# debbiemarkslab/EVcouplings

Measured on NVIDIA H100. Metric: PLM gradient evals/s as N*L^2*q cell-ops/s, higher is better.
Workload: dtype f32 parameters/accumulation; tensor-core products as bf16 hi+lo pairs (16 mantissa bits)

## Files before the change

evcouplings_b200/_lib.py:

```python
import ctypes
import os

_HERE = os.path.dirname(os.path.abspath(__file__))
LIB_PATH = os.path.join(_HERE, "csrc", "libevcplm.so")
ABI_VERSION = 2


class EngineUnavailableError(RuntimeError):
    """libevcplm.so (the sm_90a CUDA engine) is missing / unloadable / has no device."""


class EngineError(RuntimeError):
    """A libevcplm call returned non-zero."""


c_void_p = ctypes.c_void_p
c_i32 = ctypes.c_int32
c_i64 = ctypes.c_int64
c_f32 = ctypes.c_float
c_f64 = ctypes.c_double


class FitParams(ctypes.Structure):
    _fields_ = [("max_iterations", c_i32), ("m", c_i32), ("epsilon", c_f32), ("lambda_h", c_f32),
# ... 49 lines not shown
    "evc_msa_encode": (ctypes.c_int, [c_void_p, c_i64, c_i64, c_void_p, c_void_p, c_i64, c_void_p, c_void_p, c_void_p]),
    "evc_identities_to_seq": (ctypes.c_int, [c_void_p, c_void_p, c_i64, c_i32, c_void_p, c_void_p]),
    "evc_plm_create": (ctypes.c_int, [c_void_p, c_void_p, c_i64, c_i32, c_i32, c_i32, c_void_p, c_i32]),
    "evc_plm_create_alphabet": (ctypes.c_int, [c_void_p, c_void_p, c_i64, c_i32, c_i32, c_i32, c_void_p, c_i32]),
    "evc_plm_destroy": (None, [c_void_p]),
    "evc_plm_num_params": (c_i64, [c_void_p]),
    "evc_plm_eval_data": (ctypes.c_int, [c_void_p, c_void_p, c_void_p, c_void_p, c_void_p]),
    "evc_plm_set_backward": (ctypes.c_int, [c_void_p, c_i32]),
    "evc_plm_set_forward": (ctypes.c_int, [c_void_p, c_i32]),
    "evc_plm_set_precision": (ctypes.c_int, [c_void_p, c_i32]),
    "evc_plm_set_seq_chunk": (ctypes.c_int, [c_void_p, c_i64]),
    "evc_plm_tc_bytes": (ctypes.c_int, [c_i64, c_i32, c_i32, c_i32, c_i64, c_i32, c_void_p]),
    "evc_plm_tc_bytes_alphabet": (ctypes.c_int, [c_i64, c_i32, c_i32, c_i32, c_i64, c_i32, c_void_p]),
    "evc_plm_device_bytes": (c_i64, [c_void_p]),
    "evc_plm_copy_onehot": (ctypes.c_int, [c_void_p, c_void_p, c_i64]),
    "evc_fit_workspace_bytes": (c_i64, [c_i64, c_i32]),
    "evc_plm_set_host_history": (ctypes.c_int, [c_void_p, c_i32]),
    "evc_fit_workspace_split_bytes": (ctypes.c_int, [c_i64, c_i32, c_i32, c_void_p, c_void_p]),
    "evc_plm_host_bytes": (ctypes.c_int, [c_void_p, c_void_p, c_void_p]),
    "evc_fit_default_params": (None, [c_void_p]),
    "evc_plm_fit": (ctypes.c_int, [c_void_p, c_void_p, c_void_p, c_void_p, c_void_p, c_void_p, c_void_p, c_void_p,
                                   c_void_p]),
    "evc_plm_fit_checkpointed": (ctypes.c_int, [c_void_p, c_void_p, c_void_p, c_void_p, c_void_p, c_void_p, c_void_p,
                                                c_void_p, c_void_p, c_f64, c_void_p, c_void_p, c_void_p]),
    "evc_plm_fit_prepare": (ctypes.c_int, [c_void_p, c_i32]),
    "evc_plm_fit_vector": (ctypes.c_int, [c_void_p, c_i32, c_i32, c_void_p]),
    "evc_plm_pack_fx": (ctypes.c_int, [c_void_p, c_void_p, c_void_p]),
    "evc_plm_unpack_fx": (ctypes.c_int, [c_void_p, c_void_p, c_void_p]),
    "evc_plm_set_profiling": (ctypes.c_int, [c_void_p, c_i32]),
    "evc_plm_last_stage_ms": (ctypes.c_int, [c_void_p, c_void_p]),
# ... 59 lines not shown
```

evcouplings_b200/csrc/api.cu:

```cuda
#include "../../include/evcplm.h"

#include <stdlib.h>

#include <algorithm>
#include <new>
#include <string>
#include <vector>

#include "common.cuh"
#include "internal.h"

namespace evc {
static thread_local std::string g_err;
void set_error(const std::string &msg) { g_err = msg; }
}

using namespace evc;

static cudaStream_t as_stream(void *s) { return reinterpret_cast<cudaStream_t>(s); }

static const char SUPPORTED_Q[] =
    "supported: 2 <= q <= 32 states with the gap as a state, 2 <= q <= 31 with the ignored gap coded q; "
    "every code must be below 32, the 5 bit-planes of the Hamming pass";

// ... 400 lines not shown
    const bool tcf = h->fwd_mode == 1;
    const bool tcff = h->fwd_mode == 2;
    const int single = h->precision == 1 ? 1 : 0;
    void *rt_lo = single ? nullptr : h->d_rt_lo;
    float *gJ = d_g + (int64_t)g.L * g.q;
    if (tc && h->tc.n_chunks > 1) {
        if (!tcf) {
            set_error("evc_plm_eval_data: sequence chunks need the tensor-core forward (evc_plm_set_forward 1)");
            return 1;
        }
        h->ev_valid = false;
        if (plm_tcf_expand(g, h->tcf, d_x, h->d_wt_hi, h->d_wt_lo, single, st)) return 1;
        for (int c = 0; c < h->tc.n_chunks; c++) {
            const int64_t n0 = (int64_t)c * h->tc.C, nreal = std::min(h->tc.C, g.N - n0);
            if (plm_tcf_build_xsp(g, h->tcf, h->d_msa4, h->d_x1h, n0, st)) return 1;
            if (plm_tc_build_xt(g, h->tc, h->d_msa4, h->d_xt, n0, st)) return 1;
            if (plm_tcf_logits(g, h->tcf, h->tcf_maps, h->d_x1h, h->d_zt, single, nreal, st)) return 1;
            if (plm_tcf_softmax(g, h->tcf, h->d_zt, d_x, h->d_msa4, h->d_wts, h->d_rt_hi, rt_lo, h->tc.Kp,
                                h->d_gh_part2, h->d_fx_part2, n0, nreal, st))
                return 1;
            if (plm_tc_backward(g, h->tc, h->tc_maps, h->d_Gd, single, c, st)) return 1;
        }
        if (plm_tc_finalize_pairs(g, h->tc, h->d_Gd, h->tc.planes, gJ, 1.0f, st)) return 1;
        return plm_finalize_fields_n(g, h->d_gh_part2, h->d_fx_part2, d_g, d_fx, h->tcf.ntiles_s, st);
    }
    if (!tc || (!tcf && !tcff)) {
        if (require_gather_q(h, "evc_plm_eval_data") || ensure_gather(h)) return 1;
    }
    if (prof) EVC_CUDA(cudaEventRecord(h->ev[0], st));
    if (tcff) {
        if (plm_tcff_expand(g, h->tcff, d_x, h->d_wp_hi, h->d_wp_lo, single, st)) return 1;
        if (prof) EVC_CUDA(cudaEventRecord(h->ev[1], st));
        if (plm_tcff_forward(g, h->tcff, h->tcff_maps, d_x, h->d_msa4, h->d_wts, h->d_rt_hi, h->d_rt_lo, h->tc.Kp,
                             h->d_gh_part3, h->d_fx_part3, single, st))
            return 1;
        if (prof) {
            EVC_CUDA(cudaEventRecord(h->ev[2], st));
            EVC_CUDA(cudaEventRecord(h->ev[3], st));
        }
        if (plm_tc_backward(g, h->tc, h->tc_maps, h->d_Gd, single, 0, st)) return 1;
        if (prof) EVC_CUDA(cudaEventRecord(h->ev[4], st));
        if (plm_tc_finalize_pairs(g, h->tc, h->d_Gd, h->tc.planes, gJ, 1.0f, st)) return 1;
        if (plm_finalize_fields_n(g, h->d_gh_part3, h->d_fx_part3, d_g, d_fx, h->tcff.ntile_part, st)) return 1;
    } else if (tcf) {
        if (plm_tcf_expand(g, h->tcf, d_x, h->d_wt_hi, h->d_wt_lo, single, st)) return 1;
        if (prof) EVC_CUDA(cudaEventRecord(h->ev[1], st));
        if (plm_tcf_logits(g, h->tcf, h->tcf_maps, h->d_x1h, h->d_zt, single, g.N, st)) return 1;
        if (prof) EVC_CUDA(cudaEventRecord(h->ev[2], st));
        if (plm_tcf_softmax(g, h->tcf, h->d_zt, d_x, h->d_msa4, h->d_wts, h->d_rt_hi, rt_lo, h->tc.Kp,
                            h->d_gh_part2, h->d_fx_part2, 0, g.N, st))
            return 1;
        if (prof) EVC_CUDA(cudaEventRecord(h->ev[3], st));
        if (plm_tc_backward(g, h->tc, h->tc_maps, h->d_Gd, single, 0, st)) return 1;
        if (prof) EVC_CUDA(cudaEventRecord(h->ev[4], st));
        if (plm_tc_finalize_pairs(g, h->tc, h->d_Gd, h->tc.planes, gJ, 1.0f, st)) return 1;
        if (plm_finalize_fields_n(g, h->d_gh_part2, h->d_fx_part2, d_g, d_fx, h->tcf.ntiles_s, st)) return 1;
    } else {
        if (plm_expand(g, d_x, h->d_W, st)) return 1;
        if (!tc) EVC_CUDA(cudaMemsetAsync(h->d_G, 0, (size_t)g.w_floats() * sizeof(float), st));
        if (prof) EVC_CUDA(cudaEventRecord(h->ev[1], st));
        if (plm_forward(g, h->d_W, d_x, h->d_msa4, h->d_wts, h->d_R, tc ? h->d_rt_hi : nullptr,
                        tc ? h->d_rt_lo : nullptr, h->tc.Kp, h->d_gh_part, h->d_fx_part, st))
            return 1;
        if (prof) {
            EVC_CUDA(cudaEventRecord(h->ev[2], st));
            EVC_CUDA(cudaEventRecord(h->ev[3], st));
        }
        if (tc) {
            if (plm_tc_backward(g, h->tc, h->tc_maps, h->d_Gd, single, 0, st)) return 1;
            if (prof) EVC_CUDA(cudaEventRecord(h->ev[4], st));
            if (plm_tc_finalize_pairs(g, h->tc, h->d_Gd, h->tc.planes, gJ, 1.0f, st)) return 1;
            if (plm_finalize_fields(g, h->d_gh_part, h->d_fx_part, d_g, d_fx, st)) return 1;
        } else {
            if (plm_backward(g, h->d_R, h->d_perm, h->d_bstart, h->d_G, st)) return 1;
            if (prof) EVC_CUDA(cudaEventRecord(h->ev[4], st));
            if (plm_finalize(g, h->d_G, h->d_gh_part, h->d_fx_part, d_g, gJ, d_fx, 1.0f, st)) return 1;
        }
    }
    if (prof) {
        EVC_CUDA(cudaEventRecord(h->ev[5], st));
        h->ev_valid = true;
    }
    return 0;
}
// ... 8 lines not shown
        int sm_count = 0;
        EVC_CUDA(cudaDeviceGetAttribute(&sm_count, cudaDevAttrMultiProcessorCount, h->device));
        plm_tc_geometry(h->g, sm_count, h->seq_chunk, h->tc);
        const PlmTcGeom &t = h->tc;
        const TcBwdBytes b(t);
        if (!dalloc(h, &h->d_xt, b.xt) || !dalloc(h, &h->d_rt_hi, b.rt) || !dalloc(h, &h->d_rt_lo, b.rt) ||
            !dalloc(h, &h->d_Gd, b.gd)) {
            set_error(std::string("evc_plm_set_backward: device allocation failed: ") +
                      cudaGetErrorString(cudaGetLastError()));
            return 1;
        }
        EVC_CUDA(cudaMemset(h->d_xt, 0, b.xt));
        EVC_CUDA(cudaMemset(h->d_rt_hi, 0, b.rt));
        EVC_CUDA(cudaMemset(h->d_rt_lo, 0, b.rt));
        EVC_CUDA(cudaMemset(h->d_Gd, 0, b.gd));
        if (t.n_chunks == 1 && plm_tc_build_xt(h->g, t, h->d_msa4, h->d_xt, 0, 0)) return 1;
        EVC_CUDA(cudaDeviceSynchronize());
        h->tc_maps = aligned_alloc(64, round_up((int64_t)plm_tc_map_bytes(), 64));
        if (!h->tc_maps) { set_error("evc_plm_set_backward: out of host memory"); return 1; }
        if (plm_tc_make_maps(t, h->d_xt, h->d_rt_hi, h->d_rt_lo, h->tc_maps)) return 1;
    }
    h->bwd_mode = mode;
    return 0;
}

int evc_plm_set_forward(evc_plm_t *h, int32_t mode)
{
    if (!h) { set_error("evc_plm_set_forward: null handle"); return 1; }
    if (mode < 0 || mode > 2) {
        set_error("evc_plm_set_forward: mode must be 0 (gather), 1 (tensor core) or 2 (tensor core, fused softmax)");
        return 1;
    }
    if (mode == 0 && require_gather_q(h, "evc_plm_set_forward")) return 1;
    EVC_CUDA(cudaSetDevice(h->device));
    const int64_t chunk = plm_seq_chunk_round(h->seq_chunk);
// ... 119 lines not shown
int evc_plm_copy_onehot(const evc_plm_t *h, void *host_dst, int64_t bytes)
{
    if (!h || !host_dst) { set_error("evc_plm_copy_onehot: null pointer"); return 1; }
    if (!h->d_x1h) { set_error("evc_plm_copy_onehot: the handle has no tensor-core forward (evc_plm_set_forward)"); return 1; }
    const int64_t have = h->tcf.Xrows * h->tcf.Kw * 2;
    if (bytes != have) {
        set_error("evc_plm_copy_onehot: bytes must be the operand's allocation, " + std::to_string(have));
        return 1;
    }
    EVC_CUDA(cudaSetDevice(h->device));
    EVC_CUDA(cudaDeviceSynchronize());
    EVC_CUDA(cudaMemcpy(host_dst, h->d_x1h, (size_t)bytes, cudaMemcpyDeviceToHost));
    return 0;
}

int64_t evc_fit_workspace_bytes(int64_t n, int32_t m) { return n > 0 && m > 0 ? fit_work_bytes(n, m) : -1; }

int evc_fit_workspace_split_bytes(int64_t n, int32_t m, int32_t host_pairs, int64_t *device_bytes,
                                  int64_t *host_bytes)
{
    if (!device_bytes || !host_bytes) { set_error("evc_fit_workspace_split_bytes: null pointer"); return 1; }
    if (n <= 0 || m < 1 || m > 32 || host_pairs < 0 || host_pairs > m) {
        set_error("evc_fit_workspace_split_bytes: invalid arguments (need n >= 1, 1 <= m <= 32, "
                  "0 <= host_pairs <= m)");
        return 1;
    }
    fit_work_bytes(n, m, host_pairs, device_bytes, host_bytes);
    return 0;
}

// ... 67 lines not shown
    EVC_CUDA(cudaMemcpyAsync(fx_out, h->d_fx_tmp, 2 * sizeof(double), cudaMemcpyDeviceToHost, 0));
    EVC_CUDA(cudaStreamSynchronize(0));
    return 0;
}

int evc_plm_weighted_counts(evc_plm_t *h, float *d_fi_counts, float *d_fij_counts, void *stream)
{
    if (!h || !d_fi_counts || !d_fij_counts) { set_error("evc_plm_weighted_counts: null pointer"); return 1; }
    cudaStream_t st = as_stream(stream);
    const PlmGeom &g = h->g;
    if (h->bwd_mode == 1 && h->d_gh_part2) {
        const int ntiles = h->tcf.ntiles_s;
        const PlmTcGeom &t = h->tc;
        for (int c = 0; c < t.n_chunks; c++) {
            const int64_t n0 = (int64_t)c * t.C, nreal = std::min(t.C, g.N - n0);
            if (t.n_chunks > 1 && plm_tc_build_xt(g, t, h->d_msa4, h->d_xt, n0, st)) return 1;
            if (plm_tc_onehot_residual(g, ntiles, h->d_msa4, h->d_wts, h->d_rt_hi, h->d_rt_lo, t.Kp, h->d_gh_part2,
                                       h->d_fx_part2, n0, nreal, st))
                return 1;
            if (plm_tc_backward(g, t, h->tc_maps, h->d_Gd, 0, c, st)) return 1;
        }
        if (plm_tc_finalize_pairs(g, t, h->d_Gd, t.planes, d_fij_counts, 0.5f, st)) return 1;
        return plm_finalize_fields_n(g, h->d_gh_part2, nullptr, d_fi_counts, nullptr, ntiles, st);
    }
    if (require_gather_q(h, "evc_plm_weighted_counts") || ensure_gather(h)) return 1;
    EVC_CUDA(cudaMemsetAsync(h->d_G, 0, (size_t)g.w_floats() * sizeof(float), st));
    if (plm_onehot_residual(g, h->d_msa4, h->d_wts, h->d_R, h->d_gh_part, st)) return 1;
    if (plm_backward(g, h->d_R, h->d_perm, h->d_bstart, h->d_G, st)) return 1;
    return plm_finalize(g, h->d_G, h->d_gh_part, nullptr, d_fi_counts, d_fij_counts, nullptr, 0.5f, st);
}

int evc_ec_scores(const float *d_J_tri, const float *d_fij_tri, const float *d_fi, int32_t L, int32_t q,
                  float *d_fn_raw, float *d_fn_zero_sum, float *d_mi, void *stream)
{
    if (!d_J_tri) { set_error("evc_ec_scores: null pointer"); return 1; }
// ... 53 lines not shown
```

evcouplings_b200/csrc/internal.h:

```cpp
#pragma once
#include <cuda_runtime.h>
#include <stdint.h>

namespace evc {

int64_t hamming_plane_words(int64_t N, int L);
int64_t hamming_num_tiles(int64_t N);
int hamming_pack(const uint8_t *d_codes, int64_t N, int L, uint32_t *d_planes, cudaStream_t st);
int hamming_count_tiles(const uint32_t *d_planes, const int *d_mult, int64_t N, int L, int min_identical,
                        int64_t tile_begin, int64_t tile_end, int *d_counts, cudaStream_t st);

int identities_to_seq(const uint8_t *d_codes, const uint8_t *d_seq, int64_t N, int L, int *d_out, cudaStream_t st);

int msa_unique(const uint8_t *d_codes, int64_t N, int L, int *d_first, int *d_inverse, int *d_mult, int64_t *U_out,
               cudaStream_t st);

struct PlmGeom {
    int64_t N;
    int L;
    int Lp;
    int q;
    int QB;
    int S;
    int gap_code;
// ... 39 lines not shown
    int n_chunks;
    int64_t Mp;
    int64_t Np;
    int64_t Kp;
    int ksplit;
    int ksplit_last;
    int planes;
    int64_t kp_chunk(int c, int64_t N) const
    {
        const int64_t n = N - (int64_t)c * C < C ? N - (int64_t)c * C : C;
        return (n + 63) / 64 * 64;
    }
};
void plm_tc_geometry(const PlmGeom &g, int sm_count, int64_t seq_chunk, PlmTcGeom &t);
size_t plm_tc_map_bytes();
int plm_tc_build_xt(const PlmGeom &g, const PlmTcGeom &t, const uint32_t *d_msa4, void *d_xt, int64_t n0,
                    cudaStream_t st);
int plm_tc_make_maps(const PlmTcGeom &t, void *d_xt, void *d_rt_hi, void *d_rt_lo, void *maps_out_host);
int plm_tc_backward(const PlmGeom &g, const PlmTcGeom &t, const void *maps_host, float *d_Gd, int single, int chunk,
                    cudaStream_t st);
int plm_tc_onehot_residual(const PlmGeom &g, int ntiles, const uint32_t *d_msa4, const float *d_wts, void *d_rt_hi,
                           void *d_rt_lo, int64_t Kp, float *d_gh_part, double *d_fx_part, int64_t n0, int64_t nreal,
                           cudaStream_t st);
int plm_tc_finalize_pairs(const PlmGeom &g, const PlmTcGeom &t, const float *d_Gd, int planes, float *d_gJ,
                          float scale, cudaStream_t st);
struct PlmTcfGeom {
    int64_t Mp;
    int64_t Kw;
    int64_t Ns;
    int64_t Xrows;
    int ntiles_s;
};
void plm_tcf_geometry(const PlmGeom &g, const PlmTcGeom &tc, PlmTcfGeom &t);
int plm_tcf_build_x(const PlmGeom &g, const PlmTcfGeom &t, const uint32_t *d_msa4, void *d_x1h, int64_t n0,
                    cudaStream_t st);
// ... 107 lines not shown
```

evcouplings_b200/csrc/plm_tc.cu:

```cuda
#include <cuda.h>
#include <cuda_bf16.h>

#include <stdlib.h>

#include <algorithm>

#include "common.cuh"
#include "internal.h"

namespace evc {

constexpr int TC_BM = 128;
constexpr int TC_BN = 192;
constexpr int TC_BK = 64;
constexpr int TC_MAX_STAGES = 8;
constexpr int TC_A_BYTES = TC_BM * TC_BK * 2;
constexpr int TC_B_BYTES = TC_BN * TC_BK * 2;
constexpr int TC_SMEM_LIMIT = 232448;
constexpr int TC_SMEM_HEAD = 2048;
constexpr int TC_THREADS = 384;
constexpr int TC_CONSUMERS = 256;
constexpr int TC_K_CHUNK = 32;
constexpr int TC_MAX_KSPLIT = 8;
constexpr int TC_REG_PRODUCER = 40;
constexpr int TC_REG_CONSUMER = 232;

__device__ __forceinline__ void mbar_wait_bounded(uint64_t *bar, uint32_t parity)
{
    uint32_t done = 0;
    for (uint64_t it = 0; it < (1ull << 31); it++) {
        asm volatile(
            "{\n.reg .pred p;\n"
// ... 144 lines not shown
        : "+f"(d[0]), "+f"(d[1]), "+f"(d[2]), "+f"(d[3]), "+f"(d[4]), "+f"(d[5]), "+f"(d[6]), "+f"(d[7]),
          "+f"(d[8]), "+f"(d[9]), "+f"(d[10]), "+f"(d[11]), "+f"(d[12]), "+f"(d[13]), "+f"(d[14]), "+f"(d[15]),
          "+f"(d[16]), "+f"(d[17]), "+f"(d[18]), "+f"(d[19]), "+f"(d[20]), "+f"(d[21]), "+f"(d[22]), "+f"(d[23]),
          "+f"(d[24]), "+f"(d[25]), "+f"(d[26]), "+f"(d[27]), "+f"(d[28]), "+f"(d[29]), "+f"(d[30]), "+f"(d[31]),
          "+f"(d[32]), "+f"(d[33]), "+f"(d[34]), "+f"(d[35]), "+f"(d[36]), "+f"(d[37]), "+f"(d[38]), "+f"(d[39]),
          "+f"(d[40]), "+f"(d[41]), "+f"(d[42]), "+f"(d[43]), "+f"(d[44]), "+f"(d[45]), "+f"(d[46]), "+f"(d[47]),
          "+f"(d[48]), "+f"(d[49]), "+f"(d[50]), "+f"(d[51]), "+f"(d[52]), "+f"(d[53]), "+f"(d[54]), "+f"(d[55]),
          "+f"(d[56]), "+f"(d[57]), "+f"(d[58]), "+f"(d[59]), "+f"(d[60]), "+f"(d[61]), "+f"(d[62]), "+f"(d[63]),
          "+f"(d[64]), "+f"(d[65]), "+f"(d[66]), "+f"(d[67]), "+f"(d[68]), "+f"(d[69]), "+f"(d[70]), "+f"(d[71]),
          "+f"(d[72]), "+f"(d[73]), "+f"(d[74]), "+f"(d[75]), "+f"(d[76]), "+f"(d[77]), "+f"(d[78]), "+f"(d[79]),
          "+f"(d[80]), "+f"(d[81]), "+f"(d[82]), "+f"(d[83]), "+f"(d[84]), "+f"(d[85]), "+f"(d[86]), "+f"(d[87]),
          "+f"(d[88]), "+f"(d[89]), "+f"(d[90]), "+f"(d[91]), "+f"(d[92]), "+f"(d[93]), "+f"(d[94]), "+f"(d[95])
        : "r"(a.x), "r"(a.y), "r"(a.z), "r"(a.w), "l"(db), "r"(e), "r"(scale_d));
}

__device__ __forceinline__ uint4 lds128(uint32_t addr)
{
    uint4 v;
    asm volatile("ld.shared.v4.u32 {%0, %1, %2, %3}, [%4];" : "=r"(v.x), "=r"(v.y), "=r"(v.z), "=r"(v.w) : "r"(addr));
    return v;
}
__device__ __forceinline__ uint32_t lds32(uint32_t addr)
{
    uint32_t v;
    asm volatile("ld.shared.u32 %0, [%1];" : "=r"(v) : "r"(addr));
    return v;
}
__device__ __forceinline__ uint32_t cluster_ctarank()
{
    uint32_t r;
// ... 86 lines not shown
}
__device__ __forceinline__ void tc_init_barriers(const TcSmem &l, int n_stages)
{
    if (threadIdx.x == 0) {
        for (int s = 0; s < n_stages; s++) {
            mbar_init(&l.full[s], 1);
            mbar_init(&l.empty[s], TC_CONSUMERS);
        }
        mbar_fence_init();
    }
    __syncthreads();
}

template <int SINGLE, int ACC = 0>
__global__ void __launch_bounds__(TC_THREADS, 1)
tc_gemm_kernel(const __grid_constant__ CUtensorMap tm0, const __grid_constant__ CUtensorMap tm1,
               const __grid_constant__ CUtensorMap tm2, float *__restrict__ D, int64_t ldd, int m_tiles, int n_tiles,
               int num_kb, int k_chunk, int mgroup, int n_stages, int ksplit, int64_t plane, int acc_planes)
{
    constexpr int BYTES0 = TC_A_BYTES;
    constexpr int BYTES1 = TC_B_BYTES;
    constexpr int BYTES2 = TC_B_BYTES;
    constexpr int stage_bytes = BYTES0 + BYTES1 + (SINGLE ? 0 : BYTES2);
    extern __shared__ unsigned char smem_dyn[];
    const TcSmem l = tc_smem_layout(smem_dyn);
    const int tiles = m_tiles * n_tiles;
    const int slice = (int)blockIdx.x / tiles;
    int m_tile, n_tile;
    decode_tile((int)blockIdx.x - slice * tiles, m_tiles, n_tiles, mgroup, m_tile, n_tile);
    const int kb_per = (num_kb + ksplit - 1) / ksplit;
    const int kb_begin = slice * kb_per, kb_end = min(num_kb, kb_begin + kb_per);
    tc_init_barriers(l, n_stages);

    if (threadIdx.x < 128) {
        setmaxnreg_dec<TC_REG_PRODUCER>();
        if (threadIdx.x == 0) {
            int s = 0;
            uint32_t ph = 0;
            for (int kb = kb_begin; kb < kb_end; kb++) {
                mbar_wait_bounded(&l.empty[s], ph ^ 1u);
                unsigned char *st = l.ring + s * stage_bytes;
                mbar_expect_tx(&l.full[s], (uint32_t)stage_bytes);
                tma_load_2d(st, &tm0, kb * TC_BK, m_tile * TC_BM, &l.full[s]);
                tma_load_2d(st + BYTES0, &tm1, kb * TC_BK, n_tile * TC_BN, &l.full[s]);
                if (!SINGLE) tma_load_2d(st + BYTES0 + BYTES1, &tm2, kb * TC_BK, n_tile * TC_BN, &l.full[s]);
                if (++s == n_stages) { s = 0; ph ^= 1u; }
            }
        }
    } else {
        setmaxnreg_inc<TC_REG_CONSUMER>();
        const int cw = (threadIdx.x >> 7) - 1;
        constexpr uint64_t OFF1 = (uint64_t)(BYTES0 >> 4), OFF2 = (uint64_t)((BYTES0 + BYTES1) >> 4);
        const uint64_t arow = (uint64_t)((cw * 64 * TC_BK * 2) >> 4);
        const uint64_t desc0 = make_desc_sw128(l.ring);
        float acc[TC_BN / 2], sum[TC_BN / 2];
#pragma unroll
        for (int u = 0; u < TC_BN / 2; u++) acc[u] = 0.f;
        const int n_chunks = (kb_end - kb_begin + k_chunk - 1) / k_chunk;
        int s = 0;
        uint32_t ph = 0;
        for (int c = 0; c < n_chunks; c++) {
            const int kb0 = kb_begin + c * k_chunk, kb1 = min(kb_end, kb0 + k_chunk);
            tc_mainloop<TC_BN>(acc, l.full, l.empty, s, ph, n_stages, stage_bytes, kb0, kb1, desc0,
                               arow, OFF1, arow, OFF2, !SINGLE);
#pragma unroll
            for (int u = 0; u < TC_BN / 2; u++) sum[u] = (c == 0) ? acc[u] : sum[u] + acc[u];
        }
        const int t = threadIdx.x & 127;
        const int64_t row = (int64_t)m_tile * TC_BM + cw * 64 + (t >> 5) * 16 + ((t & 31) >> 2);
        float *out = D + slice * plane + row * ldd + (int64_t)n_tile * TC_BN + 2 * (t & 3);
        if (ACC && slice < acc_planes) {
#pragma unroll
            for (int c8 = 0; c8 < TC_BN / 8; c8++) {
                float2 *p0 = reinterpret_cast<float2 *>(out + 8 * c8);
                float2 *p1 = reinterpret_cast<float2 *>(out + 8 * ldd + 8 * c8);
                const float2 v0 = __ldcs(p0), v1 = __ldcs(p1);
                __stcs(p0, make_float2(v0.x + sum[4 * c8], v0.y + sum[4 * c8 + 1]));
                __stcs(p1, make_float2(v1.x + sum[4 * c8 + 2], v1.y + sum[4 * c8 + 3]));
            }
            return;
        }
#pragma unroll
        for (int c8 = 0; c8 < TC_BN / 8; c8++) {
// ... 467 lines not shown
        const float v = warp_sum(z[0][a] + z[1][a]);
        if (lane == 0) s_gh[warp * 32 + a] = v;
    }
    const double fw = warp_sum(fx_local);
    if (lane == 0) s_fx[warp] = fw;
    __syncthreads();
    if (tid < g.S) {
        float tot = 0.f;
        if (tid < q)
            for (int ww = 0; ww < 4; ww++) tot += s_gh[ww * 32 + tid];
        gh_part[((int64_t)i * ntiles + tile) * g.S + tid] = tot;
    }
    if (tid == 0) fx_part[(int64_t)i * ntiles + tile] = (s_fx[0] + s_fx[1]) + (s_fx[2] + s_fx[3]);
}

__global__ void build_xt_kernel(const uint32_t *__restrict__ msa4, __nv_bfloat16 *__restrict__ Xt, int64_t n0,
                                int64_t N, int64_t Nld, int64_t Kp, int L, int q)
{
    const int64_t n = (int64_t)blockIdx.x * blockDim.x + threadIdx.x;
    const int j = blockIdx.y;
    if (n >= Kp) return;
    int code = 255;
    if (n0 + n < N) code = (int)((msa4[(int64_t)(j >> 2) * Nld + n0 + n] >> (8 * (j & 3))) & 0xffu);
    for (int b = 0; b < q; b++)
        Xt[((int64_t)j * q + b) * Kp + n] = __float2bfloat16(code == b ? 1.0f : 0.0f);
}

constexpr int FIN_SITES = 4;
constexpr int FIN_W = FIN_SITES * 21;
constexpr int FIN_PITCH = FIN_W + 1;
constexpr int FIN_THREADS = 256;
constexpr int FIN_SMEM = 2 * FIN_W * FIN_PITCH * (int)sizeof(float);
constexpr int FIN_BATCH = 8;
static int fin_pitch(int q) { return q <= 21 ? FIN_PITCH : FIN_SITES * q + 1; }
static int fin_smem_bytes(int q) { return q <= 21 ? FIN_SMEM : 2 * (fin_pitch(q) - 1) * fin_pitch(q) * (int)sizeof(float); }

template <bool WIDE = false>
__global__ void __launch_bounds__(FIN_THREADS)
finalize_pairs_tc_kernel(const float *__restrict__ Gd, int planes, int64_t plane, float *__restrict__ gJ, int L,
                         int q, int Np, float scale, int wide_pitch)
// ... 133 lines not shown
void plm_tc_geometry(const PlmGeom &g, int sm_count, int64_t seq_chunk, PlmTcGeom &t)
{
    const int64_t lq = (int64_t)g.L * g.q;
    const int64_t c = plm_seq_chunk_round(seq_chunk);
    t.C = (c == 0 || c >= g.N) ? g.N : c;
    t.n_chunks = (int)ceil_div(g.N, t.C);
    t.Mp = round_up(lq, TC_BM);
    t.Np = round_up(lq, TC_BN);
    t.Kp = round_up(t.C, TC_BK);
    const int64_t tiles = (t.Mp / TC_BM) * (t.Np / TC_BN);
    t.ksplit = backward_ksplit(tiles, (int)(t.Kp / TC_BK), sm_count);
    t.ksplit_last = backward_ksplit(tiles, (int)(t.kp_chunk(t.n_chunks - 1, g.N) / TC_BK), sm_count);
    t.planes = std::max(t.ksplit, t.ksplit_last);
}

int plm_tc_build_xt(const PlmGeom &g, const PlmTcGeom &t, const uint32_t *d_msa4, void *d_xt, int64_t n0,
                    cudaStream_t st)
{
    dim3 grid((unsigned)ceil_div(t.Kp, 256), (unsigned)g.L);
    build_xt_kernel<<<grid, 256, 0, st>>>(d_msa4, reinterpret_cast<__nv_bfloat16 *>(d_xt), n0, g.N, g.Nld, t.Kp,
                                          g.L, g.q);
    EVC_KERNEL_CHECK();
    return 0;
}

int plm_tc_make_maps(const PlmTcGeom &t, void *d_xt, void *d_rt_hi, void *d_rt_lo, void *maps_out)
{
    CUtensorMap *m = reinterpret_cast<CUtensorMap *>(maps_out);
    if (make_map(&m[0], d_xt, t.Mp, t.Kp, TC_BM)) return 1;
    if (make_map(&m[1], d_rt_hi, t.Np, t.Kp, TC_BN)) return 1;
    if (make_map(&m[2], d_rt_lo, t.Np, t.Kp, TC_BN)) return 1;
    return 0;
}

int plm_tc_backward(const PlmGeom &g, const PlmTcGeom &t, const void *maps, float *d_Gd, int single, int chunk,
                    cudaStream_t st)
{
    const CUtensorMap *m = reinterpret_cast<const CUtensorMap *>(maps);
    const int stage = TC_A_BYTES + TC_B_BYTES + (single ? 0 : TC_B_BYTES);
    const int n_stages = stages_for(stage);
    const size_t smem = (size_t)n_stages * stage + TC_SMEM_HEAD;
    static int kc_env = -2;
    const int kc = env_int_once("EVC_KCHUNK", &kc_env);
    const int k_chunk = kc > 0 ? kc : TC_K_CHUNK;
    const int m_tiles = (int)(t.Mp / TC_BM), n_tiles = (int)(t.Np / TC_BN);
    const bool last = chunk == t.n_chunks - 1;
    const int ksplit = last ? t.ksplit_last : t.ksplit;
    const int num_kb = (int)(t.kp_chunk(chunk, g.N) / TC_BK);
    const int grid = m_tiles * n_tiles * ksplit;
    const int64_t plane = t.Mp * t.Np;
    if (chunk == 0) {
        if (single) {
            EVC_CUDA(cudaFuncSetAttribute(tc_gemm_kernel<1>, cudaFuncAttributeMaxDynamicSharedMemorySize, TC_SMEM_LIMIT));
            tc_gemm_kernel<1><<<grid, TC_THREADS, smem, st>>>(m[0], m[1], m[2], d_Gd, t.Np, m_tiles, n_tiles,
                                                                num_kb, k_chunk, m_tiles, n_stages, ksplit, plane, 0);
        } else {
            EVC_CUDA(cudaFuncSetAttribute(tc_gemm_kernel<0>, cudaFuncAttributeMaxDynamicSharedMemorySize, TC_SMEM_LIMIT));
            tc_gemm_kernel<0><<<grid, TC_THREADS, smem, st>>>(m[0], m[1], m[2], d_Gd, t.Np, m_tiles, n_tiles,
                                                                num_kb, k_chunk, m_tiles, n_stages, ksplit, plane, 0);
        }
    } else {
        const int acc_planes = t.ksplit;
        if (single) {
            EVC_CUDA(cudaFuncSetAttribute(tc_gemm_kernel<1, 1>, cudaFuncAttributeMaxDynamicSharedMemorySize, TC_SMEM_LIMIT));
            tc_gemm_kernel<1, 1><<<grid, TC_THREADS, smem, st>>>(m[0], m[1], m[2], d_Gd, t.Np, m_tiles, n_tiles,
                                                                   num_kb, k_chunk, m_tiles, n_stages, ksplit, plane,
                                                                   acc_planes);
        } else {
            EVC_CUDA(cudaFuncSetAttribute(tc_gemm_kernel<0, 1>, cudaFuncAttributeMaxDynamicSharedMemorySize, TC_SMEM_LIMIT));
            tc_gemm_kernel<0, 1><<<grid, TC_THREADS, smem, st>>>(m[0], m[1], m[2], d_Gd, t.Np, m_tiles, n_tiles,
                                                                   num_kb, k_chunk, m_tiles, n_stages, ksplit, plane,
                                                                   acc_planes);
        }
    }
    EVC_KERNEL_CHECK();
    return 0;
}

int plm_tc_finalize_pairs(const PlmGeom &g, const PlmTcGeom &t, const float *d_Gd, int planes, float *d_gJ,
                          float scale, cudaStream_t st)
{
    const unsigned nt = (unsigned)ceil_div(g.L, FIN_SITES);
    auto kernel = g.q > 21 ? finalize_pairs_tc_kernel<true> : finalize_pairs_tc_kernel<false>;
    const int smem = fin_smem_bytes(g.q);
    EVC_CUDA(cudaFuncSetAttribute(kernel, cudaFuncAttributeMaxDynamicSharedMemorySize, smem));
// ... 214 lines not shown
```

include/evcplm.h:

```cpp
#ifndef EVCPLM_H
#define EVCPLM_H

#include <stdint.h>

#ifdef __cplusplus
extern "C" {
#endif

#define EVCPLM_ABI_VERSION 2

typedef struct evc_plm evc_plm_t;

int evc_abi_version(void);
const char *evc_last_error(void);
int evc_device_count(void);
int evc_device_info(int32_t device, int32_t *sm_count, int32_t *cc_major, int32_t *cc_minor,
                    int64_t *total_mem_bytes);

int evc_hamming_counts(const uint8_t *codes, int64_t N, int32_t L, int32_t min_identical,
                       int32_t device, int32_t *counts_out);

int64_t evc_hamming_plane_words(int64_t N, int32_t L);
int64_t evc_hamming_num_tiles(int64_t N);
int evc_hamming_pack(const uint8_t *d_codes, int64_t N, int32_t L, uint32_t *d_planes, void *stream);
// ... 31 lines not shown

int evc_plm_eval_data(evc_plm_t *h, const float *d_x, float *d_g, double *d_fx, void *stream);

int evc_plm_set_backward(evc_plm_t *h, int32_t mode);
int evc_plm_set_forward(evc_plm_t *h, int32_t mode);

int evc_plm_set_precision(evc_plm_t *h, int32_t mode);

int evc_plm_set_seq_chunk(evc_plm_t *h, int64_t seq_chunk);
int evc_plm_tc_bytes(int64_t N, int32_t L, int32_t q, int32_t gap_code, int64_t seq_chunk, int32_t sm_count,
                     int64_t *bytes_out);
int evc_plm_tc_bytes_alphabet(int64_t N, int32_t L, int32_t q, int32_t gap_code, int64_t seq_chunk,
                              int32_t sm_count, int64_t *bytes_out);
int64_t evc_plm_device_bytes(const evc_plm_t *h);
int evc_plm_copy_onehot(const evc_plm_t *h, void *host_dst, int64_t bytes);
int64_t evc_fit_workspace_bytes(int64_t n, int32_t m);
int evc_plm_set_host_history(evc_plm_t *h, int32_t host_pairs);
int evc_fit_workspace_split_bytes(int64_t n, int32_t m, int32_t host_pairs, int64_t *device_bytes,
                                  int64_t *host_bytes);
int evc_plm_host_bytes(const evc_plm_t *h, int64_t *bytes_out, double *pin_seconds_out);

int evc_plm_set_profiling(evc_plm_t *h, int32_t enable);
int evc_plm_last_stage_ms(evc_plm_t *h, float *ms_out);

int evc_plm_add_regulariser(evc_plm_t *h, const float *d_x, float *d_g, double *d_fx,
                            float lambda_h, float lambda_J, void *stream);

int evc_plm_eval_host(evc_plm_t *h, const float *x, float *g, double *fx_out,
                      float lambda_h, float lambda_J);

// ... 92 lines not shown
```

Measured before the change: 4893 billion.

## Stream one-hot backward operand as packed bits and expand to registers for wgmma

The backward tensor-core GEMM used to load a dense bf16 one-hot matrix X^T through TMA as its shared-memory A operand. It now stores X^T as a bit-packed layout, built with ballot, and bulk-copies only those bits into shared memory. Consumer warps expand the bits into bf16 register fragments and issue register-A wgmma. This cuts A-operand memory traffic and shared-memory stage size by 16x, which allows more pipeline stages. In exchange it adds ALU work per k-block and replaces the old async mainloop with a per-block wait<0> loop that may serialize MMA issue.

After: 5003 billion (median of 6 runs). 1.02x the previous value.

```diff
diff --git a/evcouplings_b200/_lib.py b/evcouplings_b200/_lib.py
--- a/evcouplings_b200/_lib.py
+++ b/evcouplings_b200/_lib.py
@@ -87,6 +87,7 @@
     "evc_plm_tc_bytes_alphabet": (ctypes.c_int, [c_i64, c_i32, c_i32, c_i32, c_i64, c_i32, c_void_p]),
     "evc_plm_device_bytes": (c_i64, [c_void_p]),
     "evc_plm_copy_onehot": (ctypes.c_int, [c_void_p, c_void_p, c_i64]),
+    "evc_plm_copy_onehot_bwd": (ctypes.c_int, [c_void_p, c_void_p, c_i64]),
     "evc_fit_workspace_bytes": (c_i64, [c_i64, c_i32]),
     "evc_plm_set_host_history": (ctypes.c_int, [c_void_p, c_i32]),
     "evc_fit_workspace_split_bytes": (ctypes.c_int, [c_i64, c_i32, c_i32, c_void_p, c_void_p]),
diff --git a/evcouplings_b200/csrc/api.cu b/evcouplings_b200/csrc/api.cu
--- a/evcouplings_b200/csrc/api.cu
+++ b/evcouplings_b200/csrc/api.cu
@@ -438,12 +438,12 @@
         for (int c = 0; c < h->tc.n_chunks; c++) {
             const int64_t n0 = (int64_t)c * h->tc.C, nreal = std::min(h->tc.C, g.N - n0);
             if (plm_tcf_build_xsp(g, h->tcf, h->d_msa4, h->d_x1h, n0, st)) return 1;
-            if (plm_tc_build_xt(g, h->tc, h->d_msa4, h->d_xt, n0, st)) return 1;
+            if (plm_tc_build_xbits(g, h->tc, h->d_msa4, h->d_xt, n0, st)) return 1;
             if (plm_tcf_logits(g, h->tcf, h->tcf_maps, h->d_x1h, h->d_zt, single, nreal, st)) return 1;
             if (plm_tcf_softmax(g, h->tcf, h->d_zt, d_x, h->d_msa4, h->d_wts, h->d_rt_hi, rt_lo, h->tc.Kp,
                                 h->d_gh_part2, h->d_fx_part2, n0, nreal, st))
                 return 1;
-            if (plm_tc_backward(g, h->tc, h->tc_maps, h->d_Gd, single, c, st)) return 1;
+            if (plm_tc_backward(g, h->tc, h->tc_maps, h->d_xt, h->d_Gd, single, c, st)) return 1;
         }
         if (plm_tc_finalize_pairs(g, h->tc, h->d_Gd, h->tc.planes, gJ, 1.0f, st)) return 1;
         return plm_finalize_fields_n(g, h->d_gh_part2, h->d_fx_part2, d_g, d_fx, h->tcf.ntiles_s, st);
@@ -462,7 +462,7 @@
             EVC_CUDA(cudaEventRecord(h->ev[2], st));
             EVC_CUDA(cudaEventRecord(h->ev[3], st));
         }
-        if (plm_tc_backward(g, h->tc, h->tc_maps, h->d_Gd, single, 0, st)) return 1;
+        if (plm_tc_backward(g, h->tc, h->tc_maps, h->d_xt, h->d_Gd, single, 0, st)) return 1;
         if (prof) EVC_CUDA(cudaEventRecord(h->ev[4], st));
         if (plm_tc_finalize_pairs(g, h->tc, h->d_Gd, h->tc.planes, gJ, 1.0f, st)) return 1;
         if (plm_finalize_fields_n(g, h->d_gh_part3, h->d_fx_part3, d_g, d_fx, h->tcff.ntile_part, st)) return 1;
@@ -475,7 +475,7 @@
                             h->d_gh_part2, h->d_fx_part2, 0, g.N, st))
             return 1;
         if (prof) EVC_CUDA(cudaEventRecord(h->ev[3], st));
-        if (plm_tc_backward(g, h->tc, h->tc_maps, h->d_Gd, single, 0, st)) return 1;
+        if (plm_tc_backward(g, h->tc, h->tc_maps, h->d_xt, h->d_Gd, single, 0, st)) return 1;
         if (prof) EVC_CUDA(cudaEventRecord(h->ev[4], st));
         if (plm_tc_finalize_pairs(g, h->tc, h->d_Gd, h->tc.planes, gJ, 1.0f, st)) return 1;
         if (plm_finalize_fields_n(g, h->d_gh_part2, h->d_fx_part2, d_g, d_fx, h->tcf.ntiles_s, st)) return 1;
@@ -491,7 +491,7 @@
             EVC_CUDA(cudaEventRecord(h->ev[3], st));
         }
         if (tc) {
-            if (plm_tc_backward(g, h->tc, h->tc_maps, h->d_Gd, single, 0, st)) return 1;
+            if (plm_tc_backward(g, h->tc, h->tc_maps, h->d_xt, h->d_Gd, single, 0, st)) return 1;
             if (prof) EVC_CUDA(cudaEventRecord(h->ev[4], st));
             if (plm_tc_finalize_pairs(g, h->tc, h->d_Gd, h->tc.planes, gJ, 1.0f, st)) return 1;
             if (plm_finalize_fields(g, h->d_gh_part, h->d_fx_part, d_g, d_fx, st)) return 1;
@@ -530,11 +530,11 @@
         EVC_CUDA(cudaMemset(h->d_rt_hi, 0, b.rt));
         EVC_CUDA(cudaMemset(h->d_rt_lo, 0, b.rt));
         EVC_CUDA(cudaMemset(h->d_Gd, 0, b.gd));
-        if (t.n_chunks == 1 && plm_tc_build_xt(h->g, t, h->d_msa4, h->d_xt, 0, 0)) return 1;
+        if (t.n_chunks == 1 && plm_tc_build_xbits(h->g, t, h->d_msa4, h->d_xt, 0, 0)) return 1;
         EVC_CUDA(cudaDeviceSynchronize());
         h->tc_maps = aligned_alloc(64, round_up((int64_t)plm_tc_map_bytes(), 64));
         if (!h->tc_maps) { set_error("evc_plm_set_backward: out of host memory"); return 1; }
-        if (plm_tc_make_maps(t, h->d_xt, h->d_rt_hi, h->d_rt_lo, h->tc_maps)) return 1;
+        if (plm_tc_make_maps(t, h->d_rt_hi, h->d_rt_lo, h->tc_maps)) return 1;
     }
     h->bwd_mode = mode;
     return 0;
@@ -684,6 +684,21 @@
     return 0;
 }
 
+int evc_plm_copy_onehot_bwd(const evc_plm_t *h, void *host_dst, int64_t bytes)
+{
+    if (!h || !host_dst) { set_error("evc_plm_copy_onehot_bwd: null pointer"); return 1; }
+    if (!h->d_xt) { set_error("evc_plm_copy_onehot_bwd: the handle has no tensor-core backward (evc_plm_set_backward)"); return 1; }
+    const int64_t have = h->tc.Mp * h->tc.Kp / 8;
+    if (bytes != have) {
+        set_error("evc_plm_copy_onehot_bwd: bytes must be the operand's size, " + std::to_string(have));
+        return 1;
+    }
+    EVC_CUDA(cudaSetDevice(h->device));
+    EVC_CUDA(cudaDeviceSynchronize());
+    EVC_CUDA(cudaMemcpy(host_dst, h->d_xt, (size_t)bytes, cudaMemcpyDeviceToHost));
+    return 0;
+}
+
 int64_t evc_fit_workspace_bytes(int64_t n, int32_t m) { return n > 0 && m > 0 ? fit_work_bytes(n, m) : -1; }
 
 int evc_fit_workspace_split_bytes(int64_t n, int32_t m, int32_t host_pairs, int64_t *device_bytes,
@@ -781,11 +796,11 @@
         const PlmTcGeom &t = h->tc;
         for (int c = 0; c < t.n_chunks; c++) {
             const int64_t n0 = (int64_t)c * t.C, nreal = std::min(t.C, g.N - n0);
-            if (t.n_chunks > 1 && plm_tc_build_xt(g, t, h->d_msa4, h->d_xt, n0, st)) return 1;
+            if (t.n_chunks > 1 && plm_tc_build_xbits(g, t, h->d_msa4, h->d_xt, n0, st)) return 1;
             if (plm_tc_onehot_residual(g, ntiles, h->d_msa4, h->d_wts, h->d_rt_hi, h->d_rt_lo, t.Kp, h->d_gh_part2,
                                        h->d_fx_part2, n0, nreal, st))
                 return 1;
-            if (plm_tc_backward(g, t, h->tc_maps, h->d_Gd, 0, c, st)) return 1;
+            if (plm_tc_backward(g, t, h->tc_maps, h->d_xt, h->d_Gd, 0, c, st)) return 1;
         }
         if (plm_tc_finalize_pairs(g, t, h->d_Gd, t.planes, d_fij_counts, 0.5f, st)) return 1;
         return plm_finalize_fields_n(g, h->d_gh_part2, nullptr, d_fi_counts, nullptr, ntiles, st);
diff --git a/evcouplings_b200/csrc/internal.h b/evcouplings_b200/csrc/internal.h
--- a/evcouplings_b200/csrc/internal.h
+++ b/evcouplings_b200/csrc/internal.h
@@ -77,11 +77,11 @@
 };
 void plm_tc_geometry(const PlmGeom &g, int sm_count, int64_t seq_chunk, PlmTcGeom &t);
 size_t plm_tc_map_bytes();
-int plm_tc_build_xt(const PlmGeom &g, const PlmTcGeom &t, const uint32_t *d_msa4, void *d_xt, int64_t n0,
-                    cudaStream_t st);
-int plm_tc_make_maps(const PlmTcGeom &t, void *d_xt, void *d_rt_hi, void *d_rt_lo, void *maps_out_host);
-int plm_tc_backward(const PlmGeom &g, const PlmTcGeom &t, const void *maps_host, float *d_Gd, int single, int chunk,
-                    cudaStream_t st);
+int plm_tc_build_xbits(const PlmGeom &g, const PlmTcGeom &t, const uint32_t *d_msa4, void *d_xt, int64_t n0,
+                       cudaStream_t st);
+int plm_tc_make_maps(const PlmTcGeom &t, void *d_rt_hi, void *d_rt_lo, void *maps_out_host);
+int plm_tc_backward(const PlmGeom &g, const PlmTcGeom &t, const void *maps_host, const void *d_xt, float *d_Gd,
+                    int single, int chunk, cudaStream_t st);
 int plm_tc_onehot_residual(const PlmGeom &g, int ntiles, const uint32_t *d_msa4, const float *d_wts, void *d_rt_hi,
                            void *d_rt_lo, int64_t Kp, float *d_gh_part, double *d_fx_part, int64_t n0, int64_t nreal,
                            cudaStream_t st);
diff --git a/evcouplings_b200/csrc/plm_tc.cu b/evcouplings_b200/csrc/plm_tc.cu
--- a/evcouplings_b200/csrc/plm_tc.cu
+++ b/evcouplings_b200/csrc/plm_tc.cu
@@ -16,6 +16,7 @@
 constexpr int TC_MAX_STAGES = 8;
 constexpr int TC_A_BYTES = TC_BM * TC_BK * 2;
 constexpr int TC_B_BYTES = TC_BN * TC_BK * 2;
+constexpr int XB_KB_BYTES = TC_BM * TC_BK / 8;
 constexpr int TC_SMEM_LIMIT = 232448;
 constexpr int TC_SMEM_HEAD = 2048;
 constexpr int TC_THREADS = 384;
@@ -190,6 +191,41 @@
         : "r"(a.x), "r"(a.y), "r"(a.z), "r"(a.w), "l"(db), "r"(e), "r"(scale_d));
 }
 
+__device__ __forceinline__ void wgmma_bf16_192_ra(float *d, const uint4 &a, uint64_t db, uint32_t scale_d)
+{
+    asm volatile(
+        "{\n.reg .pred p;\n"
+        "setp.ne.b32 p, %101, 0;\n"
+        "wgmma.mma_async.sync.aligned.m64n192k16.f32.bf16.bf16 "
+        "{"
+        "%0, %1, %2, %3, %4, %5, %6, %7, %8, %9, %10, %11, %12, %13, %14, %15, "
+        "%16, %17, %18, %19, %20, %21, %22, %23, %24, %25, %26, %27, %28, %29, %30, %31, "
+        "%32, %33, %34, %35, %36, %37, %38, %39, %40, %41, %42, %43, %44, %45, %46, %47, "
+        "%48, %49, %50, %51, %52, %53, %54, %55, %56, %57, %58, %59, %60, %61, %62, %63, "
+        "%64, %65, %66, %67, %68, %69, %70, %71, %72, %73, %74, %75, %76, %77, %78, %79, "
+        "%80, %81, %82, %83, %84, %85, %86, %87, %88, %89, %90, %91, %92, %93, %94, %95"
+        "}, {%96, %97, %98, %99}, %100, p, 1, 1, 0;\n}\n"
+        : "+f"(d[0]), "+f"(d[1]), "+f"(d[2]), "+f"(d[3]), "+f"(d[4]), "+f"(d[5]), "+f"(d[6]), "+f"(d[7]),
+          "+f"(d[8]), "+f"(d[9]), "+f"(d[10]), "+f"(d[11]), "+f"(d[12]), "+f"(d[13]), "+f"(d[14]), "+f"(d[15]),
+          "+f"(d[16]), "+f"(d[17]), "+f"(d[18]), "+f"(d[19]), "+f"(d[20]), "+f"(d[21]), "+f"(d[22]), "+f"(d[23]),
+          "+f"(d[24]), "+f"(d[25]), "+f"(d[26]), "+f"(d[27]), "+f"(d[28]), "+f"(d[29]), "+f"(d[30]), "+f"(d[31]),
+          "+f"(d[32]), "+f"(d[33]), "+f"(d[34]), "+f"(d[35]), "+f"(d[36]), "+f"(d[37]), "+f"(d[38]), "+f"(d[39]),
+          "+f"(d[40]), "+f"(d[41]), "+f"(d[42]), "+f"(d[43]), "+f"(d[44]), "+f"(d[45]), "+f"(d[46]), "+f"(d[47]),
+          "+f"(d[48]), "+f"(d[49]), "+f"(d[50]), "+f"(d[51]), "+f"(d[52]), "+f"(d[53]), "+f"(d[54]), "+f"(d[55]),
+          "+f"(d[56]), "+f"(d[57]), "+f"(d[58]), "+f"(d[59]), "+f"(d[60]), "+f"(d[61]), "+f"(d[62]), "+f"(d[63]),
+          "+f"(d[64]), "+f"(d[65]), "+f"(d[66]), "+f"(d[67]), "+f"(d[68]), "+f"(d[69]), "+f"(d[70]), "+f"(d[71]),
+          "+f"(d[72]), "+f"(d[73]), "+f"(d[74]), "+f"(d[75]), "+f"(d[76]), "+f"(d[77]), "+f"(d[78]), "+f"(d[79]),
+          "+f"(d[80]), "+f"(d[81]), "+f"(d[82]), "+f"(d[83]), "+f"(d[84]), "+f"(d[85]), "+f"(d[86]), "+f"(d[87]),
+          "+f"(d[88]), "+f"(d[89]), "+f"(d[90]), "+f"(d[91]), "+f"(d[92]), "+f"(d[93]), "+f"(d[94]), "+f"(d[95])
+        : "r"(a.x), "r"(a.y), "r"(a.z), "r"(a.w), "l"(db), "r"(scale_d));
+}
+
+__device__ __forceinline__ uint32_t onehot_pair(uint32_t v, int s)
+{
+    const uint32_t b = (v >> s) & 3u;
+    return ((b * 0x8001u) & 0x10001u) * 0x3F80u;
+}
+
 __device__ __forceinline__ uint4 lds128(uint32_t addr)
 {
     uint4 v;
@@ -306,14 +342,14 @@
 
 template <int SINGLE, int ACC = 0>
 __global__ void __launch_bounds__(TC_THREADS, 1)
-tc_gemm_kernel(const __grid_constant__ CUtensorMap tm0, const __grid_constant__ CUtensorMap tm1,
-               const __grid_constant__ CUtensorMap tm2, float *__restrict__ D, int64_t ldd, int m_tiles, int n_tiles,
-               int num_kb, int k_chunk, int mgroup, int n_stages, int ksplit, int64_t plane, int acc_planes)
-{
-    constexpr int BYTES0 = TC_A_BYTES;
-    constexpr int BYTES1 = TC_B_BYTES;
-    constexpr int BYTES2 = TC_B_BYTES;
-    constexpr int stage_bytes = BYTES0 + BYTES1 + (SINGLE ? 0 : BYTES2);
+tc_gemm_kernel(const __grid_constant__ CUtensorMap tm_hi, const __grid_constant__ CUtensorMap tm_lo,
+               const unsigned char *__restrict__ xbits, int kb_stride, float *__restrict__ D, int64_t ldd,
+               int m_tiles, int n_tiles, int num_kb, int k_chunk, int mgroup, int n_stages, int ksplit, int64_t plane,
+               int acc_planes)
+{
+    constexpr int OFF_A = TC_B_BYTES;
+    constexpr int OFF_LO = TC_B_BYTES + XB_KB_BYTES;
+    constexpr int stage_bytes = OFF_LO + (SINGLE ? 0 : TC_B_BYTES);
     extern __shared__ unsigned char smem_dyn[];
     const TcSmem l = tc_smem_layout(smem_dyn);
     const int tiles = m_tiles * n_tiles;
@@ -327,24 +363,27 @@
     if (threadIdx.x < 128) {
         setmaxnreg_dec<TC_REG_PRODUCER>();
         if (threadIdx.x == 0) {
+            const unsigned char *src = xbits + (int64_t)m_tile * kb_stride * XB_KB_BYTES;
             int s = 0;
             uint32_t ph = 0;
             for (int kb = kb_begin; kb < kb_end; kb++) {
                 mbar_wait_bounded(&l.empty[s], ph ^ 1u);
                 unsigned char *st = l.ring + s * stage_bytes;
                 mbar_expect_tx(&l.full[s], (uint32_t)stage_bytes);
-                tma_load_2d(st, &tm0, kb * TC_BK, m_tile * TC_BM, &l.full[s]);
-                tma_load_2d(st + BYTES0, &tm1, kb * TC_BK, n_tile * TC_BN, &l.full[s]);
-                if (!SINGLE) tma_load_2d(st + BYTES0 + BYTES1, &tm2, kb * TC_BK, n_tile * TC_BN, &l.full[s]);
+                tma_load_2d(st, &tm_hi, kb * TC_BK, n_tile * TC_BN, &l.full[s]);
+                bulk_g2s(st + OFF_A, src + (int64_t)kb * XB_KB_BYTES, XB_KB_BYTES, &l.full[s]);
+                if (!SINGLE) tma_load_2d(st + OFF_LO, &tm_lo, kb * TC_BK, n_tile * TC_BN, &l.full[s]);
                 if (++s == n_stages) { s = 0; ph ^= 1u; }
             }
         }
     } else {
         setmaxnreg_inc<TC_REG_CONSUMER>();
         const int cw = (threadIdx.x >> 7) - 1;
-        constexpr uint64_t OFF1 = (uint64_t)(BYTES0 >> 4), OFF2 = (uint64_t)((BYTES0 + BYTES1) >> 4);
-        const uint64_t arow = (uint64_t)((cw * 64 * TC_BK * 2) >> 4);
+        const int t = threadIdx.x & 127;
+        const uint32_t a_addr = smem_u32(l.ring) + OFF_A + 16 * (8 * (4 * cw + (t >> 5)) + ((t & 31) >> 2));
+        const int kshift = 2 * (t & 3);
         const uint64_t desc0 = make_desc_sw128(l.ring);
+        constexpr uint64_t DLO = (uint64_t)(OFF_LO >> 4);
         float acc[TC_BN / 2], sum[TC_BN / 2];
 #pragma unroll
         for (int u = 0; u < TC_BN / 2; u++) acc[u] = 0.f;
@@ -353,12 +392,35 @@
         uint32_t ph = 0;
         for (int c = 0; c < n_chunks; c++) {
             const int kb0 = kb_begin + c * k_chunk, kb1 = min(kb_end, kb0 + k_chunk);
-            tc_mainloop<TC_BN>(acc, l.full, l.empty, s, ph, n_stages, stage_bytes, kb0, kb1, desc0,
-                               arow, OFF1, arow, OFF2, !SINGLE);
+            for (int kb = kb0; kb < kb1; kb++) {
+                mbar_wait_bounded(&l.full[s], ph);
+                const uint4 bits = lds128(a_addr + (uint32_t)(s * stage_bytes));
+                const uint32_t w[4] = {bits.x >> kshift, bits.y >> kshift, bits.z >> kshift, bits.w >> kshift};
+                uint4 a[TC_BK / 16];
+#pragma unroll
+                for (int k = 0; k < TC_BK / 16; k++) {
+                    const uint32_t r0 = w[k >> 1], r8 = w[2 + (k >> 1)];
+                    const int sh = 16 * (k & 1);
+                    a[k] = make_uint4(onehot_pair(r0, sh), onehot_pair(r8, sh), onehot_pair(r0, sh + 8),
+                                      onehot_pair(r8, sh + 8));
+                }
+                wgmma_fence();
+                const uint64_t d = desc0 + (uint64_t)((s * stage_bytes) >> 4);
+#pragma unroll
+                for (int k = 0; k < TC_BK / 16; k++) {
+                    const uint64_t koff = (uint64_t)((k * 16 * 2) >> 4);
+                    wgmma_bf16_192_ra(acc, a[k], d + koff, (kb == kb0 && k == 0) ? 0u : 1u);
+                    if (!SINGLE) wgmma_bf16_192_ra(acc, a[k], d + DLO + koff, 1u);
+                }
+                wgmma_commit();
+                wgmma_wait<0>();
+                mbar_arrive(&l.empty[s]);
+                if (++s == n_stages) { s = 0; ph ^= 1u; }
+            }
+            fence_regs<TC_BN / 2>(acc);
 #pragma unroll
             for (int u = 0; u < TC_BN / 2; u++) sum[u] = (c == 0) ? acc[u] : sum[u] + acc[u];
         }
-        const int t = threadIdx.x & 127;
         const int64_t row = (int64_t)m_tile * TC_BM + cw * 64 + (t >> 5) * 16 + ((t & 31) >> 2);
         float *out = D + slice * plane + row * ldd + (int64_t)n_tile * TC_BN + 2 * (t & 3);
         if (ACC && slice < acc_planes) {
@@ -856,16 +918,33 @@
     if (tid == 0) fx_part[(int64_t)i * ntiles + tile] = (s_fx[0] + s_fx[1]) + (s_fx[2] + s_fx[3]);
 }
 
-__global__ void build_xt_kernel(const uint32_t *__restrict__ msa4, __nv_bfloat16 *__restrict__ Xt, int64_t n0,
-                                int64_t N, int64_t Nld, int64_t Kp, int L, int q)
-{
-    const int64_t n = (int64_t)blockIdx.x * blockDim.x + threadIdx.x;
-    const int j = blockIdx.y;
-    if (n >= Kp) return;
-    int code = 255;
-    if (n0 + n < N) code = (int)((msa4[(int64_t)(j >> 2) * Nld + n0 + n] >> (8 * (j & 3))) & 0xffu);
-    for (int b = 0; b < q; b++)
-        Xt[((int64_t)j * q + b) * Kp + n] = __float2bfloat16(code == b ? 1.0f : 0.0f);
+__global__ void __launch_bounds__(256)
+build_xbits_kernel(const uint32_t *__restrict__ msa4, uint32_t *__restrict__ out, int64_t n0, int64_t N,
+                   int64_t Nld, int L, int q, int kb_stride)
+{
+    const int kb = blockIdx.x, T = blockIdx.y;
+    const int lane = threadIdx.x & 31, w = threadIdx.x >> 5, h = w & 1;
+    const int64_t n = n0 + (int64_t)kb * TC_BK + 32 * h + lane;
+    const bool real = n < N;
+    const int rt0 = 32 * (w >> 1), row0 = T * TC_BM + rt0;
+    auto code_of = [&](int j) -> int {
+        return (real && j < L) ? (int)((msa4[(int64_t)(j >> 2) * Nld + n] >> (8 * (j & 3))) & 0xffu) : 255;
+    };
+    int j = row0 / q, b = row0 - j * q;
+    int code = code_of(j);
+    uint32_t mine = 0;
+#pragma unroll 4
+    for (int i = 0; i < 32; i++) {
+        const uint32_t m = __ballot_sync(0xffffffffu, code == b);
+        if (lane == i) mine = m;
+        if (++b == q) {
+            b = 0;
+            code = code_of(++j);
+        }
+    }
+    const int rt = rt0 + lane;
+    uint32_t *blk = out + ((int64_t)T * kb_stride + kb) * (XB_KB_BYTES / 4);
+    blk[4 * (8 * (rt >> 4) + (rt & 7)) + 2 * ((rt >> 3) & 1) + h] = mine;
 }
 
 constexpr int FIN_SITES = 4;
@@ -1029,30 +1108,31 @@
     t.planes = std::max(t.ksplit, t.ksplit_last);
 }
 
-int plm_tc_build_xt(const PlmGeom &g, const PlmTcGeom &t, const uint32_t *d_msa4, void *d_xt, int64_t n0,
-                    cudaStream_t st)
-{
-    dim3 grid((unsigned)ceil_div(t.Kp, 256), (unsigned)g.L);
-    build_xt_kernel<<<grid, 256, 0, st>>>(d_msa4, reinterpret_cast<__nv_bfloat16 *>(d_xt), n0, g.N, g.Nld, t.Kp,
-                                          g.L, g.q);
+int plm_tc_build_xbits(const PlmGeom &g, const PlmTcGeom &t, const uint32_t *d_msa4, void *d_xt, int64_t n0,
+                       cudaStream_t st)
+{
+    const int kbs = (int)(t.Kp / TC_BK);
+    build_xbits_kernel<<<dim3((unsigned)kbs, (unsigned)(t.Mp / TC_BM)), 256, 0, st>>>(
+        d_msa4, reinterpret_cast<uint32_t *>(d_xt), n0, g.N, g.Nld, g.L, g.q, kbs);
     EVC_KERNEL_CHECK();
     return 0;
 }
 
-int plm_tc_make_maps(const PlmTcGeom &t, void *d_xt, void *d_rt_hi, void *d_rt_lo, void *maps_out)
+int plm_tc_make_maps(const PlmTcGeom &t, void *d_rt_hi, void *d_rt_lo, void *maps_out)
 {
     CUtensorMap *m = reinterpret_cast<CUtensorMap *>(maps_out);
-    if (make_map(&m[0], d_xt, t.Mp, t.Kp, TC_BM)) return 1;
-    if (make_map(&m[1], d_rt_hi, t.Np, t.Kp, TC_BN)) return 1;
-    if (make_map(&m[2], d_rt_lo, t.Np, t.Kp, TC_BN)) return 1;
+    if (make_map(&m[0], d_rt_hi, t.Np, t.Kp, TC_BN)) return 1;
+    if (make_map(&m[1], d_rt_lo, t.Np, t.Kp, TC_BN)) return 1;
     return 0;
 }
 
-int plm_tc_backward(const PlmGeom &g, const PlmTcGeom &t, const void *maps, float *d_Gd, int single, int chunk,
-                    cudaStream_t st)
+int plm_tc_backward(const PlmGeom &g, const PlmTcGeom &t, const void *maps, const void *d_xt, float *d_Gd,
+                    int single, int chunk, cudaStream_t st)
 {
     const CUtensorMap *m = reinterpret_cast<const CUtensorMap *>(maps);
-    const int stage = TC_A_BYTES + TC_B_BYTES + (single ? 0 : TC_B_BYTES);
+    const unsigned char *xb = reinterpret_cast<const unsigned char *>(d_xt);
+    const int kbs = (int)(t.Kp / TC_BK);
+    const int stage = TC_B_BYTES + XB_KB_BYTES + (single ? 0 : TC_B_BYTES);
     const int n_stages = stages_for(stage);
     const size_t smem = (size_t)n_stages * stage + TC_SMEM_HEAD;
     static int kc_env = -2;
@@ -1067,23 +1147,23 @@
     if (chunk == 0) {
         if (single) {
             EVC_CUDA(cudaFuncSetAttribute(tc_gemm_kernel<1>, cudaFuncAttributeMaxDynamicSharedMemorySize, TC_SMEM_LIMIT));
-            tc_gemm_kernel<1><<<grid, TC_THREADS, smem, st>>>(m[0], m[1], m[2], d_Gd, t.Np, m_tiles, n_tiles,
+            tc_gemm_kernel<1><<<grid, TC_THREADS, smem, st>>>(m[0], m[1], xb, kbs, d_Gd, t.Np, m_tiles, n_tiles,
                                                                 num_kb, k_chunk, m_tiles, n_stages, ksplit, plane, 0);
         } else {
             EVC_CUDA(cudaFuncSetAttribute(tc_gemm_kernel<0>, cudaFuncAttributeMaxDynamicSharedMemorySize, TC_SMEM_LIMIT));
-            tc_gemm_kernel<0><<<grid, TC_THREADS, smem, st>>>(m[0], m[1], m[2], d_Gd, t.Np, m_tiles, n_tiles,
+            tc_gemm_kernel<0><<<grid, TC_THREADS, smem, st>>>(m[0], m[1], xb, kbs, d_Gd, t.Np, m_tiles, n_tiles,
                                                                 num_kb, k_chunk, m_tiles, n_stages, ksplit, plane, 0);
         }
     } else {
         const int acc_planes = t.ksplit;
         if (single) {
             EVC_CUDA(cudaFuncSetAttribute(tc_gemm_kernel<1, 1>, cudaFuncAttributeMaxDynamicSharedMemorySize, TC_SMEM_LIMIT));
-            tc_gemm_kernel<1, 1><<<grid, TC_THREADS, smem, st>>>(m[0], m[1], m[2], d_Gd, t.Np, m_tiles, n_tiles,
+            tc_gemm_kernel<1, 1><<<grid, TC_THREADS, smem, st>>>(m[0], m[1], xb, kbs, d_Gd, t.Np, m_tiles, n_tiles,
                                                                    num_kb, k_chunk, m_tiles, n_stages, ksplit, plane,
                                                                    acc_planes);
         } else {
             EVC_CUDA(cudaFuncSetAttribute(tc_gemm_kernel<0, 1>, cudaFuncAttributeMaxDynamicSharedMemorySize, TC_SMEM_LIMIT));
-            tc_gemm_kernel<0, 1><<<grid, TC_THREADS, smem, st>>>(m[0], m[1], m[2], d_Gd, t.Np, m_tiles, n_tiles,
+            tc_gemm_kernel<0, 1><<<grid, TC_THREADS, smem, st>>>(m[0], m[1], xb, kbs, d_Gd, t.Np, m_tiles, n_tiles,
                                                                    num_kb, k_chunk, m_tiles, n_stages, ksplit, plane,
                                                                    acc_planes);
         }
diff --git a/include/evcplm.h b/include/evcplm.h
--- a/include/evcplm.h
+++ b/include/evcplm.h
@@ -69,6 +69,7 @@
                               int32_t sm_count, int64_t *bytes_out);
 int64_t evc_plm_device_bytes(const evc_plm_t *h);
 int evc_plm_copy_onehot(const evc_plm_t *h, void *host_dst, int64_t bytes);
+int evc_plm_copy_onehot_bwd(const evc_plm_t *h, void *host_dst, int64_t bytes);
 int64_t evc_fit_workspace_bytes(int64_t n, int32_t m);
 int evc_plm_set_host_history(evc_plm_t *h, int32_t host_pairs);
 int evc_fit_workspace_split_bytes(int64_t n, int32_t m, int32_t host_pairs, int64_t *device_bytes,
```
